# feiyue126/find_circ2

Measured on AMD Instinct MI355X. Metric: anchor-pairs/sec (backsplice calls) at 100 bp reads, 1/2/4/8 MI355X, higher is better.
Workload: dtype u32

## Files before the change

### find_circ2_amd/csrc/fc2_inflate.hip

```cpp
#include <hip/hip_runtime.h>
#include <stdint.h>
#include <string.h>

#include <algorithm>
#include <atomic>
#include <mutex>
#include <string>
#include <vector>

#include "../../include/fc2_ingest.h"
#include "fc2_common.h"
#include "fc2_devcrc.h"
#include "fc2_inflate.h"

namespace {

constexpr uint32_t kOutMax = 65536;
constexpr uint32_t kRing = 16384;
constexpr uint32_t kRingMask = kRing - 1;
constexpr uint32_t kFlush = 4096;
constexpr int kLitBits = 9;
constexpr int kDistBits = 7;

enum : uint32_t { INF_OK = 0, INF_BAD_TYPE = 1, INF_BAD_STORED = 2, INF_BAD_COUNTS = 3, INF_BAD_CODE = 4,
                  INF_BAD_DIST = 5, INF_OVERFLOW = 6, INF_OVERRUN = 7, INF_SHORT = 8, INF_TOO_BIG = 9,
                  INF_BAD_CLCODE = 10, INF_BAD_CLSYM = 11, INF_BAD_REPEAT = 12, INF_NO_EOB = 13,
                  INF_BAD_LITCODE = 14, INF_BAD_DISTCODE = 15, INF_BAD_CRC = 16 };

enum : uint32_t { K_LIT = 0, K_LEN = 1, K_EOB = 2, K_BAD = 3 };
enum Table { T_LIT, T_DIST, T_CL };

__device__ __forceinline__ uint32_t entry(uint32_t len, uint32_t extra, uint32_t kind, uint32_t value) {
    return len | (extra << 4) | (kind << 8) | (value << 16);
}

struct Lds {
    uint8_t ring[kRing];
    uint32_t lfast[1 << kLitBits];
    uint32_t dfast[1 << kDistBits];
    uint32_t cnt[16];
    uint16_t lsym[288], dsym[32];
    uint8_t lens[320];
};

__constant__ uint16_t kLBase[29] = {3, 4, 5, 6, 7, 8, 9, 10, 11, 13, 15, 17, 19, 23, 27, 31, 35, 43, 51, 59,
                                    67, 83, 99, 115, 131, 163, 195, 227, 258};
__constant__ uint8_t kLExt[29] = {0, 0, 0, 0, 0, 0, 0, 0, 1, 1, 1, 1, 2, 2, 2, 2, 3, 3, 3, 3, 4, 4, 4, 4, 5, 5, 5, 5, 0};
__constant__ uint16_t kDBase[30] = {1, 2, 3, 4, 5, 7, 9, 13, 17, 25, 33, 49, 65, 97, 129, 193, 257, 385, 513, 769,
                                    1025, 1537, 2049, 3073, 4097, 6145, 8193, 12289, 16385, 24577};
__constant__ uint8_t kDExt[30] = {0, 0, 0, 0, 1, 1, 2, 2, 3, 3, 4, 4, 5, 5, 6, 6, 7, 7, 8, 8, 9, 9, 10, 10, 11, 11,
                                  12, 12, 13, 13};
__constant__ uint8_t kClOrder[19] = {16, 17, 18, 0, 8, 7, 9, 6, 10, 5, 11, 4, 12, 3, 13, 2, 14, 1, 15};

__device__ __forceinline__ uint32_t meaning(Table t, uint32_t s, uint32_t len) {
    if (t == T_CL) return entry(len, 0, K_LIT, s);
    if (t == T_DIST) return s < 30 ? entry(len, kDExt[s], K_LEN, kDBase[s]) : entry(len, 0, K_BAD, 0);
    if (s < 256) return entry(len, 0, K_LIT, s);
    if (s == 256) return entry(len, 0, K_EOB, 0);
    return s < 286 ? entry(len, kLExt[s - 257], K_LEN, kLBase[s - 257]) : entry(len, 0, K_BAD, 0);
}

__device__ __forceinline__ uint32_t uni(uint32_t v) { return (uint32_t)__builtin_amdgcn_readfirstlane((int)v); }

struct Bits {
    const uint32_t *w;
    uint32_t pos, end;
    uint64_t bb;
    int nb;
    uint32_t wi;
    uint32_t base, last;
    uint32_t win, nxt;
    int lane;
};

__device__ __forceinline__ uint32_t load_word(const Bits &b, uint32_t k) { return k <= b.last ? b.w[k] : 0u; }
__device__ __forceinline__ void window(Bits &b, uint32_t base) {
    b.base = base;
    b.win = load_word(b, base + (uint32_t)b.lane);
    b.nxt = load_word(b, base + 64u + (uint32_t)b.lane);
}
__device__ __forceinline__ uint32_t word(Bits &b, uint32_t k) {
    if (k - b.base >= 64u) {
        if (k - b.base < 128u) {
            b.base += 64u;
            b.win = b.nxt;
            b.nxt = load_word(b, b.base + 64u + (uint32_t)b.lane);
        } else {
            window(b, k & ~63u);
        }
    }
    return (uint32_t)__builtin_amdgcn_readlane((int)b.win, (int)(k - b.base));
}
__device__ __forceinline__ void seek(Bits &b, uint32_t bitpos) {
    b.pos = bitpos;
    b.wi = bitpos >> 5;
    const uint32_t sh = bitpos & 31u;
    const uint32_t lo = word(b, b.wi);
    const uint32_t hi = word(b, b.wi + 1);
    b.bb = ((uint64_t)lo | ((uint64_t)hi << 32)) >> sh;
    b.nb = 64 - (int)sh;
    b.wi += 2;
}
__device__ __forceinline__ uint32_t peek(Bits &b) {
    if (b.nb <= 32) {
        b.bb |= (uint64_t)word(b, b.wi++) << b.nb;
        b.nb += 32;
    }
    return (uint32_t)b.bb;
}
__device__ __forceinline__ void drop(Bits &b, int n) {
    b.bb >>= n;
    b.nb -= n;
    b.pos += (uint32_t)n;
}
__device__ __forceinline__ uint32_t bits(Bits &b, int n) {
    const uint32_t v = peek(b) & ((1u << n) - 1u);
    drop(b, n);
    return v;
}

struct CodeV {
    uint32_t cnt, first, index;
};

template <int F>
__device__ __forceinline__ uint32_t decode(Bits &b, const uint32_t *fast, const CodeV &cv, const uint16_t *sym, Table t,
                                           uint32_t &val) {
    const uint32_t v = peek(b);
    uint32_t e = uni(fast[v & ((1u << F) - 1u)]);
    if (!(e & 15u)) {
        e = 0;
        const uint32_t rv = __builtin_bitreverse32(v);
        for (int l = F + 1; l <= 15; ++l) {
            const uint32_t code = rv >> (32 - l);
            const uint32_t f = (uint32_t)__builtin_amdgcn_readlane((int)cv.first, l);
            if (code - f < (uint32_t)__builtin_amdgcn_readlane((int)cv.cnt, l)) {
                const uint32_t k = (uint32_t)__builtin_amdgcn_readlane((int)cv.index, l) + code - f;
                e = meaning(t, uni(sym[k]), (uint32_t)l);
                break;
            }
        }
        if (!e) return 0;
    }
    const int cl = (int)(e & 15u), ex = (int)((e >> 4) & 15u);
    val = (e >> 16) + ((uint32_t)(b.bb >> cl) & ((1u << ex) - 1u));
    drop(b, cl + ex);
    return e;
}

template <int F>
__device__ bool build(const uint8_t *lens, int n, uint32_t *fast, uint32_t *cnt, uint16_t *sym, Table t, int lane,
                      CodeV &cv) {
    if (lane < 16) cnt[lane] = 0;
    for (int i = lane; i < (1 << F); i += 64) fast[i] = 0;
    __syncthreads();
    for (int s = lane; s < n; s += 64) {
        const uint32_t l = lens[s];
        if (l) atomicAdd(&cnt[l], 1u);
    }
    __syncthreads();
    uint32_t cnt_v = lane < 16 ? cnt[lane] : 0u;
    cnt_v = lane == 0 ? 0u : cnt_v;
    cv.cnt = cnt_v;
    uint32_t start[16], next[16];
    int left = 1;
    uint32_t idx = 0, code = 0;
#pragma unroll
    for (int l = 1; l < 16; ++l) {
        const uint32_t nl = (uint32_t)__builtin_amdgcn_readlane((int)cnt_v, l);
        const uint32_t np = (uint32_t)__builtin_amdgcn_readlane((int)cnt_v, l - 1);
        left = (left << 1) - (int)nl;
        code = (code + np) << 1;
        start[l] = idx;
        next[l] = code;
        if (lane == l) {
            cv.first = code;
            cv.index = idx;
        }
        idx += nl;
    }
    const uint32_t n1 = (uint32_t)__builtin_amdgcn_readlane((int)cnt_v, 1);
    if (left < 0 || (left > 0 && idx > n1)) {
        __syncthreads();
        return false;
    }
    for (int base = 0; base < n; base += 64) {
        const int s = base + lane;
        const uint32_t l = s < n ? lens[s] : 0u;
#pragma unroll
        for (int ll = 1; ll < 16; ++ll) {
            const uint64_t m = __ballot(l == (uint32_t)ll);
            if (!m) continue;
            if (l == (uint32_t)ll) {
                const uint32_t r = (uint32_t)__popcll(m & ((1ull << lane) - 1ull));
                sym[start[ll] + r] = (uint16_t)s;
                if (ll <= F) {
                    const uint32_t c = next[ll] + r;
                    const uint32_t rev = __builtin_bitreverse32(c) >> (32 - ll);
                    const uint32_t e = meaning(t, (uint32_t)s, (uint32_t)ll);
                    for (uint32_t k = rev; k < (1u << F); k += 1u << ll) fast[k] = e;
                }
            }
            const uint32_t c = (uint32_t)__popcll(m);
            start[ll] += c;
            next[ll] += c;
        }
    }
    __syncthreads();
    return true;
}

__device__ void flush(const Lds &L, uint8_t *dst, uint32_t &flushed, uint32_t upto, bool all, int lane, uint32_t &R) {
    __syncthreads();
    const uint32_t limit = all ? upto : flushed + (upto - flushed) / kFlush * kFlush;
    const uint32_t o = 16u * (uint32_t)lane;
    while (limit - flushed >= 1024u) {
        const uint4 v = *reinterpret_cast<const uint4 *>(L.ring + (flushed & kRingMask) + o);
        *reinterpret_cast<uint4 *>(dst + flushed + o) = v;
        const uint32_t c = crc_word(crc_word(crc_word(crc_word(0u, v.x), v.y), v.z), v.w);
        R = multmodp(kX2n[13], R) ^ wave_fold(c);
        flushed += 1024u;
    }
    if (all && upto > flushed) {
        const uint32_t t = upto - flushed, r = flushed & kRingMask;
        if (o < t) *reinterpret_cast<uint4 *>(dst + flushed + o) = *reinterpret_cast<const uint4 *>(L.ring + r + o);
        for (uint32_t i = 0; i < t; ++i) {
            R ^= uni(L.ring[r + i]);
#pragma unroll
            for (int b = 0; b < 8; ++b) R = mulx(R);
        }
        flushed = upto;
    }
    __threadfence_block();
}

__global__ __launch_bounds__(64) void inflate_kernel(const uint8_t *__restrict__ src, const uint32_t *__restrict__ off,
                                                     const uint32_t *__restrict__ len,
                                                     const uint32_t *__restrict__ isize,
                                                     const uint32_t *__restrict__ crc, uint8_t *__restrict__ dst,
                                                     uint32_t *__restrict__ status) {
    extern __shared__ __align__(16) uint8_t smem[];
    Lds &L = *reinterpret_cast<Lds *>(smem);
    const uint32_t blk = blockIdx.x;
    const int lane = (int)threadIdx.x;
    const uint32_t o = off[blk], want = isize[blk];
    uint8_t *out = dst + (uint64_t)blk * kOutMax;
    uint32_t st = INF_OK;
    if (want > kOutMax || len[blk] >= (1u << 28)) st = INF_TOO_BIG;
    const uint32_t n = st == INF_OK ? len[blk] : 0u;
    Bits b;
    b.w = reinterpret_cast<const uint32_t *>(src + (o & ~3u));
    b.end = (o & 3u) * 8u + n * 8u;
    b.last = ((o & 3u) + n) >> 2;
    b.lane = lane;
    window(b, 0);
    seek(b, (o & 3u) * 8u);
    uint32_t p = 0, flushed = 0;
    uint32_t R = 0;
    CodeV lcv = {0, 0, 0}, dcv = {0, 0, 0};
    bool last = false;
    while (st == INF_OK && !last) {
        if (b.pos + 3 > b.end) { st = INF_OVERRUN; break; }
        last = bits(b, 1) != 0;
        const uint32_t type = bits(b, 2);
        if (type == 0) {
            seek(b, (b.pos + 7u) & ~7u);
            if (b.pos + 32 > b.end) { st = INF_OVERRUN; break; }
            const uint32_t sl = bits(b, 16), nl = bits(b, 16);
            if (sl != (~nl & 0xFFFFu)) { st = INF_BAD_STORED; break; }
            if (b.pos + sl * 8u > b.end) { st = INF_OVERRUN; break; }
            if (p + sl > want) { st = INF_OVERFLOW; break; }
            const uint8_t *s = reinterpret_cast<const uint8_t *>(b.w) + (b.pos >> 3);
            for (uint32_t done = 0; done < sl;) {
                const uint32_t k = min(sl - done, kFlush);
                for (uint32_t j = (uint32_t)lane; j < k; j += 64) L.ring[(p + j) & kRingMask] = s[done + j];
                p += k;
                done += k;
                if (p - flushed >= kFlush) flush(L, out, flushed, p, false, lane, R);
            }
            seek(b, b.pos + sl * 8u);
            continue;
        }
        if (type == 3) { st = INF_BAD_TYPE; break; }
        if (type == 1) {
            for (int s = lane; s < 288 + 32; s += 64)
                L.lens[s] = (uint8_t)(s < 144 ? 8 : s < 256 ? 9 : s < 280 ? 7 : s < 288 ? 8 : 5);
            __syncthreads();
            if (!build<kLitBits>(L.lens, 288, L.lfast, L.cnt, L.lsym, T_LIT, lane, lcv) ||
                !build<kDistBits>(L.lens + 288, 32, L.dfast, L.cnt, L.dsym, T_DIST, lane, dcv)) {
                st = INF_BAD_LITCODE;
                break;
            }
        } else {
            if (b.pos + 14 > b.end) { st = INF_OVERRUN; break; }
            const int nlen = (int)bits(b, 5) + 257, ndist = (int)bits(b, 5) + 1, ncode = (int)bits(b, 4) + 4;
            if (nlen > 286 || ndist > 30) { st = INF_BAD_COUNTS; break; }
            if (lane < 19) L.lens[lane] = 0;
            __syncthreads();
            for (int k = 0; k < ncode; ++k) {
                const uint32_t v = bits(b, 3);
                if (lane == 0) L.lens[kClOrder[k]] = (uint8_t)v;
            }
            __syncthreads();
            if (!build<7>(L.lens, 19, L.dfast, L.cnt, L.dsym, T_CL, lane, dcv)) { st = INF_BAD_CLCODE; break; }
            const int total = nlen + ndist;
            int k = 0;
            while (k < total) {
                if (b.pos > b.end) { st = INF_OVERRUN; break; }
                uint32_t sym;
                if (!decode<7>(b, L.dfast, dcv, L.dsym, T_CL, sym)) { st = INF_BAD_CLSYM; break; }
                if (sym < 16) {
                    if (lane == 0) L.lens[k] = (uint8_t)sym;
                    ++k;
                    continue;
                }
                uint32_t val = 0;
                int rep;
                if (sym == 16) {
                    if (k == 0) { st = INF_BAD_REPEAT; break; }
                    __syncthreads();
                    val = uni(L.lens[k - 1]);
                    rep = 3 + (int)bits(b, 2);
                } else if (sym == 17) {
                    rep = 3 + (int)bits(b, 3);
                } else {
                    rep = 11 + (int)bits(b, 7);
                }
                if (k + rep > total) { st = INF_BAD_REPEAT; break; }
                for (int r = lane; r < rep; r += 64) L.lens[k + r] = (uint8_t)val;
                k += rep;
            }
            if (st != INF_OK) break;
            if (b.pos > b.end) { st = INF_OVERRUN; break; }
            __syncthreads();
            if (uni(L.lens[256]) == 0) { st = INF_NO_EOB; break; }
            if (!build<kLitBits>(L.lens, nlen, L.lfast, L.cnt, L.lsym, T_LIT, lane, lcv)) {
                st = INF_BAD_LITCODE;
                break;
            }
            if (!build<kDistBits>(L.lens + nlen, ndist, L.dfast, L.cnt, L.dsym, T_DIST, lane, dcv)) {
                st = INF_BAD_DISTCODE;
                break;
            }
        }
        for (;;) {
            if (b.pos > b.end) { st = INF_OVERRUN; break; }
            uint32_t val;
            const uint32_t e = decode<kLitBits>(b, L.lfast, lcv, L.lsym, T_LIT, val);
            const uint32_t kind = (e >> 8) & 0xFFu;
            if (!e || kind == K_BAD) { st = INF_BAD_CODE; break; }
            if (kind == K_LIT) {
                if (p >= want) { st = INF_OVERFLOW; break; }
                if (lane == 0) L.ring[p & kRingMask] = (uint8_t)val;
                ++p;
            } else if (kind == K_EOB) {
                break;
            } else {
                const uint32_t mlen = val;
                uint32_t dist;
                const uint32_t de = decode<kDistBits>(b, L.dfast, dcv, L.dsym, T_DIST, dist);
                if (!de || ((de >> 8) & 0xFFu) == K_BAD || dist > p) { st = INF_BAD_DIST; break; }
                if (p + mlen > want) { st = INF_OVERFLOW; break; }
                if (dist + mlen <= kRing) {
                    for (uint32_t j = (uint32_t)lane; j < mlen; j += 64)
                        L.ring[(p + j) & kRingMask] = L.ring[(p - dist + (j < dist ? j : j % dist)) & kRingMask];
                } else {
                    for (uint32_t j = (uint32_t)lane; j < mlen; j += 64)
                        L.ring[(p + j) & kRingMask] = out[p - dist + (j < dist ? j : j % dist)];
                }
                p += mlen;
            }
            if (p - flushed >= kFlush) flush(L, out, flushed, p, false, lane, R);
        }
    }
    if (st == INF_OK && p != want) st = INF_SHORT;
    if (st == INF_OK && b.pos > b.end) st = INF_OVERRUN;
    if (st == INF_OK) {
        flush(L, out, flushed, p, true, lane, R);
        if (crc && (R ^ multmodp(x8n(want), 0xFFFFFFFFu) ^ 0xFFFFFFFFu) != crc[blk]) st = INF_BAD_CRC;
    }
    if (lane == 0) status[blk] = st;
}

__global__ __launch_bounds__(256) void compact_kernel(const uint8_t *__restrict__ slots, const uint32_t *__restrict__ isize,
                                                      const uint32_t *__restrict__ ooff,
                                                      const uint32_t *__restrict__ status, uint8_t *__restrict__ out) {
    const uint32_t blk = blockIdx.y;
    const uint32_t b0 = 16u * (blockIdx.x * 256u + threadIdx.x);
    const uint32_t n = isize[blk];
    if (status[blk] != INF_OK || b0 >= n) return;
    const uint4 v = *reinterpret_cast<const uint4 *>(slots + (uint64_t)blk * kOutMax + b0);
    uint8_t *d = out + ooff[blk] + b0;
    if (b0 + 16u <= n && ((uintptr_t)d & 15u) == 0) {
        *reinterpret_cast<uint4 *>(d) = v;
        return;
    }
    const uint32_t w[4] = {v.x, v.y, v.z, v.w};
    const uint32_t k = min(16u, n - b0);
    for (uint32_t i = 0; i < k; ++i) d[i] = (uint8_t)(w[i >> 2] >> (8u * (i & 3u)));
}


constexpr uint32_t kWalkCap = FC2_BAM_WALK_CAP;
static_assert((kOutMax - 4) / 36 + 1 <= kWalkCap, "a block's record starts fit a row");

__device__ __forceinline__ uint32_t walk_u32(const uint32_t *__restrict__ w, uint32_t o) {
    const uint32_t i = o >> 2, s = (o & 3u) * 8u;
    const uint32_t lo = w[i];
    if (!s) return lo;
    return (lo >> s) | (w[i + 1] << (32u - s));
}

__device__ bool walk_plausible(const uint32_t *__restrict__ w, uint32_t o, uint32_t n) {
    if (o > n || n - o < 36u) return false;
    const uint32_t avail = n - o;
    const int32_t bs = (int32_t)walk_u32(w, o);
    if (bs < 32 || bs >= (1 << 28)) return false;
    const int32_t ref = (int32_t)walk_u32(w, o + 4), pos = (int32_t)walk_u32(w, o + 8);
    const uint32_t lname = walk_u32(w, o + 12) & 0xFFu, ncig = walk_u32(w, o + 16) & 0xFFFFu;
    const int32_t lseq = (int32_t)walk_u32(w, o + 20), nref = (int32_t)walk_u32(w, o + 24),
                  npos = (int32_t)walk_u32(w, o + 28);
    if (ref < -1 || pos < -1 || lname < 1 || lseq < 0 || nref < -1 || npos < -1) return false;
    if (32ull + lname + 4ull * ncig + ((uint64_t)lseq + 1) / 2 + (uint64_t)lseq > (uint64_t)bs) return false;
    if (36u + lname > avail) return true;
    const uint8_t *p = reinterpret_cast<const uint8_t *>(w) + o + 36u;
    if (p[lname - 1] != 0) return false;
    for (uint32_t k = 0; k + 1 < lname; ++k)
        if (p[k] < 0x21 || p[k] > 0x7e) return false;
    return true;
}

__global__ __launch_bounds__(64) void bam_walk_kernel(const uint8_t *__restrict__ slots, const uint32_t *__restrict__ isize,
                                                      const uint32_t *__restrict__ status, uint16_t *__restrict__ starts,
                                                      uint32_t *__restrict__ count, uint32_t *__restrict__ exit_at) {
    const uint32_t blk = blockIdx.x, lane = threadIdx.x;
    if (status && status[blk] != INF_OK) {
        if (lane == 0) count[blk] = 0, exit_at[blk] = FC2_BAM_WALK_NO_EXIT;
        return;
    }
    const uint32_t n = min(isize[blk], kOutMax);
    const uint32_t *w = reinterpret_cast<const uint32_t *>(slots + (uint64_t)blk * kOutMax);
    uint16_t *row = starts + (uint64_t)blk * kWalkCap;
    uint32_t o = FC2_BAM_WALK_NO_EXIT;
    for (uint32_t b = 0; b + 36u <= n; b += 64u) {
        const uint32_t c = b + lane;
        bool ok = walk_plausible(w, c, n);
        if (ok) {
            const uint32_t nx = c + 4u + walk_u32(w, c);
            ok = nx + 36u > n || walk_plausible(w, nx, n);
        }
        const unsigned long long m = __ballot(ok);
        if (m) {
            o = b + (uint32_t)__ffsll(m) - 1u;
            break;
        }
    }
    o = uni(o);
    uint32_t cnt = 0, ex = FC2_BAM_WALK_NO_EXIT;
    if (o != FC2_BAM_WALK_NO_EXIT) {
        bool cut = false;
        while (cnt < kWalkCap && o + 4u <= n) {
            const int32_t bs = (int32_t)uni(walk_u32(w, o));
            if (bs < 32) { cut = true; break; }
            if (lane == 0) row[cnt] = (uint16_t)o;
            ++cnt;
            o += 4u + (uint32_t)bs;
        }
        if (!cut) ex = o;
    }
    if (lane == 0) count[blk] = cnt, exit_at[blk] = ex;
}


constexpr uint32_t kDigestMaxBlocks = FC2_BAM_DIGEST_MAX_BLOCKS;
static_assert(sizeof(fc2_bam_digest) == 32, "a digest row is 32 bytes");

__device__ __forceinline__ uint32_t dg_u8(const uint8_t *__restrict__ b, uint64_t o) { return b[o]; }
__device__ __forceinline__ uint32_t dg_u16(const uint8_t *__restrict__ b, uint64_t o) {
    return dg_u8(b, o) | (dg_u8(b, o + 1) << 8);
}
__device__ __forceinline__ uint32_t dg_u32(const uint8_t *__restrict__ b, uint64_t o) {
    return dg_u8(b, o) | (dg_u8(b, o + 1) << 8) | (dg_u8(b, o + 2) << 16) | (dg_u8(b, o + 3) << 24);
}

__device__ __forceinline__ uint32_t dg_tag_bits(const uint8_t *__restrict__ b, uint64_t p, uint32_t ty) {
    switch (ty) {
        case 'c': return (uint32_t)(int32_t)(int8_t)dg_u8(b, p);
        case 'C': return dg_u8(b, p);
        case 's': return (uint32_t)(int32_t)(int16_t)dg_u16(b, p);
        case 'S': return dg_u16(b, p);
        case 'i': case 'I': case 'f': return dg_u32(b, p);
        default: return 0;
    }
}

__device__ bool digest_record(const uint8_t *__restrict__ bytes, uint32_t n_bytes, uint64_t at,
                              const uint32_t *__restrict__ ooff, const uint32_t *__restrict__ status, uint32_t blk,
                              uint32_t n_blocks, fc2_bam_digest &r) {
    if (at + 4 > n_bytes) return false;
    const uint32_t bs = dg_u32(bytes, at);
    r.block_size = bs;
    if (bs < 32u || bs >= (1u << 28)) return false;
    const uint64_t b = at + 4, lim = b + bs;
    if (lim > n_bytes) return false;
    if (status)
        for (uint32_t j = blk; j < n_blocks && (j == blk || ooff[j] < lim); ++j)
            if (status[j] != INF_OK) return false;
    const int64_t pos = (int32_t)dg_u32(bytes, b + 4);
    const uint32_t l_name = dg_u8(bytes, b + 8), n_cig = dg_u16(bytes, b + 12), flag = dg_u16(bytes, b + 14);
    const int64_t l_seq = (int32_t)dg_u32(bytes, b + 16);
    if (l_seq < 0 || 32 + (int64_t)l_name + 4 * (int64_t)n_cig + (l_seq + 1) / 2 + l_seq > (int64_t)bs) return false;
    if (l_name == 0 || dg_u8(bytes, b + 32 + l_name - 1) != 0) return false;
    uint64_t p = b + 32 + l_name;
    uint64_t ref_span = 0, astart = 0, lead = 0, trail = 0;
    bool stop = false, leading = true;
    for (uint32_t k = 0; k < n_cig; ++k, p += 4) {
        const uint32_t c = dg_u32(bytes, p), op = c & 0xFu, len = c >> 4;
        if (op == 0 || op == 2 || op == 3 || op == 7 || op == 8) ref_span += len;
        if (!stop) {
            if (op == 4 || op == 5) astart += len;
            else if (op == 0) stop = true;
        }
        if (leading) {
            if (op == 4) lead += len;
            else if (op != 5) leading = false;
        }
        if (op == 4) trail += len;
        else if (op != 5) trail = 0;
    }
    if ((ref_span | astart | lead | trail) >> 31) return false;
    r.astart = (int32_t)astart;
    r.aend = ((flag & 4u) || n_cig == 0) ? -1 : pos + (int64_t)ref_span;
    if (l_seq > 0) {
        const int64_t n = l_seq;
        int64_t s0 = (int64_t)lead, e0 = n - (int64_t)trail;
        if (e0 < 0) e0 += n;
        s0 = s0 > n ? n : s0;
        e0 = e0 < 0 ? 0 : (e0 > n ? n : e0);
        r.qlen = (int32_t)(e0 > s0 ? e0 - s0 : 0);
        r.has_qual = dg_u8(bytes, p + (uint64_t)(l_seq + 1) / 2) != 0xFFu;
    } else {
        r.qlen = -1;
        r.has_qual = 0;
    }
    p += (uint64_t)(l_seq + 1) / 2 + (uint64_t)l_seq;
    uint32_t n_as = 0, n_xs = 0;
    while (p < lim) {
        if (lim - p < 3) return false;
        const uint32_t t0 = dg_u8(bytes, p), t1 = dg_u8(bytes, p + 1), ty = dg_u8(bytes, p + 2);
        p += 3;
        const uint64_t left = lim - p;
        uint64_t n;
        switch (ty) {
            case 'c': case 'C': case 'A': n = 1; break;
            case 's': case 'S': n = 2; break;
            case 'i': case 'I': case 'f': n = 4; break;
            case 'Z': case 'H': {
                uint64_t z = p;
                while (z < lim && dg_u8(bytes, z) != 0) ++z;
                if (z == lim) return false;
                n = z - p + 1;
                break;
            }
            case 'B': {
                if (left < 5) return false;
                const uint32_t sub = dg_u8(bytes, p);
                const uint32_t w = (sub == 'c' || sub == 'C') ? 1u : (sub == 's' || sub == 'S') ? 2u
                                 : (sub == 'i' || sub == 'I' || sub == 'f') ? 4u : 0u;
                const int32_t cnt = (int32_t)dg_u32(bytes, p + 1);
                if (!w || cnt < 0) return false;
                n = 5 + (uint64_t)w * (uint32_t)cnt;
                break;
            }
            default: return false;
        }
        if (n > left) return false;
        const bool as = t0 == 'A' && t1 == 'S', xs = t0 == 'X' && t1 == 'S';
        if (as) {
            if (n_as++) return false;
            r.as_type = (uint8_t)ty;
            r.as_bits = dg_tag_bits(bytes, p, ty);
        }
        if (xs) {
            if (n_xs++) return false;
            r.xs_type = (uint8_t)ty;
            r.xs_bits = dg_tag_bits(bytes, p, ty);
        }
        p += n;
    }
    return true;
}

__global__ __launch_bounds__(64) void bam_digest_kernel(const uint8_t *__restrict__ bytes, uint32_t n_bytes,
                                                        const uint32_t *__restrict__ ooff, const uint32_t *__restrict__ status,
                                                        const uint16_t *__restrict__ starts, const uint32_t *__restrict__ count,
                                                        fc2_bam_digest *__restrict__ rows, uint32_t *__restrict__ first,
                                                        uint32_t n_blocks) {
    const uint32_t blk = blockIdx.x, lane = threadIdx.x;
    uint32_t f = 0;
    for (uint32_t j = lane; j < blk; j += 64u) f += min(count[j], kWalkCap);
    for (int d = 32; d; d >>= 1) f += __shfl_xor(f, d, 64);
    const uint32_t cnt = min(count[blk], kWalkCap);
    if (lane == 0) {
        first[blk] = f;
        if (blk + 1 == n_blocks) first[n_blocks] = f + cnt;
    }
    const uint16_t *row = starts + (uint64_t)blk * kWalkCap;
    const uint32_t o0 = ooff[blk];
    for (uint32_t k = lane; k < cnt; k += 64u) {
        fc2_bam_digest r;
        r.state = r.as_type = r.xs_type = r.has_qual = 0;
        r.block_size = 0;
        r.astart = r.qlen = 0;
        r.as_bits = r.xs_bits = 0;
        r.aend = 0;
        if (digest_record(bytes, n_bytes, (uint64_t)o0 + row[k], ooff, status, blk, n_blocks, r)) {
            r.state = 1;
        } else {
            const uint32_t bs = r.block_size;
            r.as_type = r.xs_type = r.has_qual = 0;
            r.astart = r.qlen = 0;
            r.as_bits = r.xs_bits = 0;
            r.aend = 0;
            r.block_size = bs;
        }
        rows[(uint64_t)f + k] = r;
    }
}

}

extern "C" int fc2_bam_digest_launch(const uint8_t *bytes, uint32_t n_bytes, const uint32_t *ooff, const uint32_t *isize,
                                     const uint32_t *status, const uint16_t *starts, const uint32_t *count,
                                     fc2_bam_digest *rows, uint32_t *first, uint32_t n_blocks, void *stream) {
    if (!n_blocks) return FC2_OK;
    if ((!bytes && n_bytes) || !ooff || !isize || !starts || !count || !rows || !first)
        return fc2::fail(FC2_E_PARAM, "fc2_bam_digest_launch: null argument");
    if (n_blocks > kDigestMaxBlocks) return fc2::fail(FC2_E_PARAM, "fc2_bam_digest_launch: more than 1024 blocks");
    if (((uintptr_t)rows & 7u) || ((uintptr_t)first & 3u))
        return fc2::fail(FC2_E_PARAM, "fc2_bam_digest_launch: rows must be 8-byte and first 4-byte aligned");
    hipLaunchKernelGGL(bam_digest_kernel, dim3(n_blocks), dim3(64), 0, (hipStream_t)stream, bytes, n_bytes, ooff, status,
                       starts, count, rows, first, n_blocks);
    const hipError_t e = hipGetLastError();
    return e == hipSuccess ? FC2_OK : fc2::fail(FC2_E_HIP, std::string("fc2_bam_digest_launch: ") + hipGetErrorString(e));
}

extern "C" int fc2_bam_walk_launch(const uint8_t *slots, const uint32_t *isize, const uint32_t *status, uint16_t *starts,
                                   uint32_t *count, uint32_t *exit, uint32_t n_blocks, void *stream) {
    if (!n_blocks) return FC2_OK;
    if (!slots || !isize || !starts || !count || !exit) return fc2::fail(FC2_E_PARAM, "fc2_bam_walk_launch: null argument");
    if ((uintptr_t)slots & 3u) return fc2::fail(FC2_E_PARAM, "fc2_bam_walk_launch: slots must be 4-byte aligned");
    hipLaunchKernelGGL(bam_walk_kernel, dim3(n_blocks), dim3(64), 0, (hipStream_t)stream, slots, isize, status, starts,
                       count, exit);
    const hipError_t e = hipGetLastError();
    return e == hipSuccess ? FC2_OK : fc2::fail(FC2_E_HIP, std::string("fc2_bam_walk_launch: ") + hipGetErrorString(e));
}

extern "C" int fc2_bgzf_inflate_launch(const uint8_t *src, const uint32_t *off, const uint32_t *len,
                                       const uint32_t *isize, const uint32_t *crc, uint8_t *dst, uint32_t *status,
                                       uint32_t n, void *stream) {
    if (!n) return FC2_OK;
    if (!src || !off || !len || !isize || !dst || !status) return fc2::fail(FC2_E_PARAM, "fc2_bgzf_inflate_launch: null argument");
    static bool attr = [] {
        return hipFuncSetAttribute(reinterpret_cast<const void *>(inflate_kernel),
                                   hipFuncAttributeMaxDynamicSharedMemorySize, (int)sizeof(Lds)) == hipSuccess;
    }();
    if (!attr) return fc2::fail(FC2_E_HIP, "fc2_bgzf_inflate_launch: cannot reserve the kernel's LDS");
    hipLaunchKernelGGL(inflate_kernel, dim3(n), dim3(64), sizeof(Lds), (hipStream_t)stream, src, off, len, isize, crc,
                       dst, status);
    const hipError_t e = hipGetLastError();
    return e == hipSuccess ? FC2_OK : fc2::fail(FC2_E_HIP, std::string("fc2_bgzf_inflate_launch: ") + hipGetErrorString(e));
}

namespace fc2 {
namespace inf {

namespace {
struct Pool {
    struct Buf {
        void *p;
        size_t size;
    };
    std::mutex mu;
    size_t cap = 0;
    int users = 0, max_buffers = 0;
    std::vector<Buf> idle, all;
};
Pool &pool() {
    static Pool *p = new Pool();
    return *p;
}
std::atomic<bool> pool_on{false};

void pool_open(size_t cap, int max_buffers) {
    Pool &P = pool();
    std::lock_guard<std::mutex> g(P.mu);
    ++P.users;
    P.cap = std::max(P.cap, cap);
    P.max_buffers = std::max(P.max_buffers, max_buffers);
    pool_on = true;
}
void pool_drop(Pool &P, void *b) {
    (void)hipHostFree(b);
    for (size_t k = 0; k < P.all.size(); ++k)
        if (P.all[k].p == b) {
            P.all.erase(P.all.begin() + (ptrdiff_t)k);
            break;
        }
}
void pool_close() {
    Pool &P = pool();
    std::lock_guard<std::mutex> g(P.mu);
    if (--P.users > 0) return;
    pool_on = false;
    for (const Pool::Buf &b : P.idle) pool_drop(P, b.p);
    P.idle.clear();
    P.cap = 0;
    P.max_buffers = 0;
}
}

void *pinned_take(size_t n) {
    if (!pool_on.load(std::memory_order_relaxed)) return nullptr;
    Pool &P = pool();
    std::lock_guard<std::mutex> g(P.mu);
    if (!P.users || n > P.cap) return nullptr;
    for (size_t k = 0; k < P.idle.size(); ++k)
        if (P.idle[k].size >= n) {
            void *b = P.idle[k].p;
            P.idle.erase(P.idle.begin() + (ptrdiff_t)k);
            return b;
        }
    if ((int)P.all.size() >= P.max_buffers) return nullptr;
    void *b = nullptr;
    if (hipHostMalloc(&b, P.cap, hipHostMallocDefault) != hipSuccess) return nullptr;
    P.all.push_back({b, P.cap});
    return b;
}

bool pinned_owns(const void *b) {
    Pool &P = pool();
    std::lock_guard<std::mutex> g(P.mu);
    for (const Pool::Buf &x : P.all)
        if (x.p == b) return true;
    return false;
}

bool pinned_give(void *b) {
    Pool &P = pool();
    std::lock_guard<std::mutex> g(P.mu);
    for (const Pool::Buf &x : P.all)
        if (x.p == b) {
            if (P.users) P.idle.push_back(x);
            else pool_drop(P, b);
            return true;
        }
    return false;
}

constexpr int kStreams = 4;

struct Gpu {
    int device = 0;
    uint32_t max_blocks = 0;
    size_t src_cap = 0;
    hipStream_t stream[kStreams] = {};
    hipEvent_t done[kStreams] = {};
    uint8_t *h_src = nullptr, *d_src = nullptr, *d_slots = nullptr, *d_out = nullptr;
    uint32_t *h_meta = nullptr, *d_meta = nullptr;
    uint32_t *h_walk = nullptr, *d_walk = nullptr;
    uint16_t *h_starts = nullptr, *d_starts = nullptr;
    bool walk = false;
    fc2_bam_digest *d_rows = nullptr, *h_rows = nullptr;
    uint32_t *d_first = nullptr, *h_first = nullptr;
    size_t rows_cap = 0;
    struct Chunk {
        uint32_t i0, c, foff;
        int s;
        uint64_t row0;
    };
    std::vector<Chunk> dchunks;
    bool digest = false, digest_ok = false, rows_ready = false;
    bool pooled = false;
    char *dest = nullptr;
    uint32_t n = 0;
    uint64_t out = 0;
    int chunks = 0;
    bool ok = true;
    std::string err;
};

static bool hip_ok(Gpu *g, hipError_t e, const char *what) {
    if (e == hipSuccess) return true;
    if (g->ok) g->err = std::string("GPU inflate: ") + what + ": " + hipGetErrorString(e);
    g->ok = false;
    return false;
}

Gpu *gpu_open(int device, uint32_t max_blocks, size_t pool_cap, std::string &err) {
    Gpu *g = new Gpu();
    g->device = device;
    g->max_blocks = max_blocks;
    g->src_cap = (size_t)max_blocks * kOutMax + 64;
    const size_t out = (size_t)max_blocks * kOutMax, meta = (size_t)max_blocks * 7 * sizeof(uint32_t);
    const size_t walk = (size_t)max_blocks * 2 * sizeof(uint32_t), rows = (size_t)max_blocks * kWalkCap * sizeof(uint16_t);
    bool ok = hip_ok(g, hipSetDevice(device), "hipSetDevice");
    for (int k = 0; k < kStreams && ok; ++k)
        ok = hip_ok(g, hipStreamCreateWithFlags(&g->stream[k], hipStreamNonBlocking), "stream") &&
             hip_ok(g, hipEventCreateWithFlags(&g->done[k], hipEventBlockingSync | hipEventDisableTiming), "event");
    ok = ok && hip_ok(g, hipHostMalloc((void **)&g->h_src, g->src_cap, hipHostMallocDefault), "pinned input") &&
         hip_ok(g, hipHostMalloc((void **)&g->h_meta, meta, hipHostMallocDefault), "pinned table") &&
         hip_ok(g, hipMalloc((void **)&g->d_src, g->src_cap), "device input") &&
         hip_ok(g, hipMalloc((void **)&g->d_slots, out), "device slots") &&
         hip_ok(g, hipMalloc((void **)&g->d_out, out), "device output") &&
         hip_ok(g, hipMalloc((void **)&g->d_meta, meta), "device table") &&
         hip_ok(g, hipHostMalloc((void **)&g->h_walk, walk, hipHostMallocDefault), "pinned record counts") &&
         hip_ok(g, hipHostMalloc((void **)&g->h_starts, rows, hipHostMallocDefault), "pinned record lists") &&
         hip_ok(g, hipMalloc((void **)&g->d_walk, walk), "device record counts") &&
         hip_ok(g, hipMalloc((void **)&g->d_starts, rows), "device record lists");
    if (!ok) {
        err = g->err;
        gpu_close(g);
        return nullptr;
    }
    if (pool_cap) {
        pool_open(pool_cap, 16);
        g->pooled = true;
        void *first[3];
        for (void *&b : first) b = pinned_take(pool_cap);
        for (void *b : first)
            if (b) pinned_give(b);
    }
    return g;
}

void gpu_close(Gpu *g) {
    if (!g) return;
    if (hipSetDevice(g->device) == hipSuccess) {
        for (int k = 0; k < kStreams; ++k)
            if (g->stream[k]) (void)hipStreamSynchronize(g->stream[k]);
        if (g->d_first) (void)hipFree(g->d_first);
        if (g->d_rows) (void)hipFree(g->d_rows);
        if (g->h_first) (void)hipHostFree(g->h_first);
        if (g->h_rows) (void)hipHostFree(g->h_rows);
        if (g->d_starts) (void)hipFree(g->d_starts);
        if (g->d_walk) (void)hipFree(g->d_walk);
        if (g->h_starts) (void)hipHostFree(g->h_starts);
        if (g->h_walk) (void)hipHostFree(g->h_walk);
        if (g->d_meta) (void)hipFree(g->d_meta);
        if (g->d_out) (void)hipFree(g->d_out);
        if (g->d_slots) (void)hipFree(g->d_slots);
        if (g->d_src) (void)hipFree(g->d_src);
        if (g->h_meta) (void)hipHostFree(g->h_meta);
        if (g->h_src) (void)hipHostFree(g->h_src);
        for (int k = 0; k < kStreams; ++k) {
            if (g->done[k]) (void)hipEventDestroy(g->done[k]);
            if (g->stream[k]) (void)hipStreamDestroy(g->stream[k]);
        }
    }
    if (g->pooled) pool_close();
    delete g;
}

uint32_t gpu_max_blocks(const Gpu *g) { return g->max_blocks; }

constexpr size_t kRowsPerBlock = 512;

void gpu_begin(Gpu *g, char *dest, bool walk, bool digest) {
    g->dest = dest;
    g->walk = walk;
    g->digest = walk && digest;
    g->digest_ok = g->digest;
    g->rows_ready = false;
    g->dchunks.clear();
    g->n = 0;
    g->out = 0;
    g->chunks = 0;
    g->ok = hipSetDevice(g->device) == hipSuccess;
    g->err = g->ok ? "" : "GPU inflate: hipSetDevice failed";
    if (g->ok && g->digest && !g->d_rows) {
        const size_t M = g->max_blocks;
        g->rows_cap = M * kRowsPerBlock;
        hip_ok(g, hipMalloc((void **)&g->d_rows, M * kWalkCap * sizeof(fc2_bam_digest)), "device digest rows") &&
            hip_ok(g, hipMalloc((void **)&g->d_first, (2 * M + 1) * sizeof(uint32_t)), "device row index") &&
            hip_ok(g, hipHostMalloc((void **)&g->h_rows, g->rows_cap * sizeof(fc2_bam_digest), hipHostMallocDefault),
                   "pinned digest rows") &&
            hip_ok(g, hipHostMalloc((void **)&g->h_first, (2 * M + 1) * sizeof(uint32_t), hipHostMallocDefault),
                   "pinned row index");
    }
}

bool gpu_add(Gpu *g, const uint8_t *raw, const size_t *boff, const size_t *bsz, size_t i0, size_t i1) {
    if (!g->ok) return false;
    if (i1 <= i0) return true;
    if (i0 != g->n || i1 > g->max_blocks || boff[i1 - 1] + bsz[i1 - 1] + 8 > g->src_cap) {
        g->ok = false;
        g->err = "GPU inflate: chunk out of order or larger than the buffers";
        return false;
    }
    const uint32_t M = g->max_blocks;
    uint32_t *off = g->h_meta, *len = off + M, *isz = len + M, *crc = isz + M, *ooff = crc + M, *st = ooff + M,
             *rooff = st + M;
    const size_t b0 = boff[i0], b1 = boff[i1 - 1] + bsz[i1 - 1];
    memcpy(g->h_src + b0, raw + b0, b1 - b0);
    memset(g->h_src + b1, 0, 8);
    bool fits = true;
    for (size_t i = i0; i < i1; ++i) {
        const uint8_t *b = raw + boff[i];
        const size_t xl = b[10] | (b[11] << 8);
        off[i] = (uint32_t)(boff[i] + 12 + xl);
        len[i] = (uint32_t)(bsz[i] - 12 - xl - 8);
        const uint8_t *t = b + bsz[i] - 8;
        crc[i] = t[0] | (t[1] << 8) | (t[2] << 16) | ((uint32_t)t[3] << 24);
        isz[i] = t[4] | (t[5] << 8) | (t[6] << 16) | ((uint32_t)t[7] << 24);
        ooff[i] = (uint32_t)g->out;
        rooff[i] = ooff[i] - ooff[i0];
        if (isz[i] > kOutMax) fits = false;
        g->out += std::min<uint32_t>(isz[i], kOutMax);
    }
    g->n = (uint32_t)i1;
    const uint32_t c = (uint32_t)(i1 - i0);
    if (!fits) {
        for (size_t i = i0; i < i1; ++i) st[i] = INF_TOO_BIG;
        g->digest_ok = false;
        return true;
    }
    hipStream_t s = g->stream[g->chunks++ % kStreams];
    uint32_t *d_off = g->d_meta, *d_len = d_off + M, *d_isz = d_len + M, *d_crc = d_isz + M, *d_ooff = d_crc + M,
             *d_st = d_ooff + M;
    const size_t w = sizeof(uint32_t);
    bool ok = hip_ok(g, hipMemcpyAsync(g->d_src + b0, g->h_src + b0, b1 + 8 - b0, hipMemcpyHostToDevice, s), "upload");
    for (int a = 0; a < 5 && ok; ++a)
        ok = hip_ok(g, hipMemcpyAsync(g->d_meta + (size_t)a * M + i0, g->h_meta + (size_t)a * M + i0, c * w,
                                      hipMemcpyHostToDevice, s), "upload");
    ok = ok && fc2_bgzf_inflate_launch(g->d_src, d_off + i0, d_len + i0, d_isz + i0, d_crc + i0,
                                       g->d_slots + (size_t)i0 * kOutMax, d_st + i0, c, s) == FC2_OK;
    if (!ok) {
        if (g->ok) g->err = "GPU inflate: launch failed";
        g->ok = false;
        return false;
    }
    hipLaunchKernelGGL(compact_kernel, dim3(kOutMax / 16 / 256, c), dim3(256), 0, s, g->d_slots + (size_t)i0 * kOutMax,
                       d_isz + i0, d_ooff + i0, d_st + i0, g->d_out);
    const uint64_t o0 = ooff[i0];
    if (!hip_ok(g, hipGetLastError(), "compact")) return false;
    if (g->walk) {
        if (fc2_bam_walk_launch(g->d_slots + (size_t)i0 * kOutMax, d_isz + i0, d_st + i0, g->d_starts + (size_t)i0 * kWalkCap,
                                g->d_walk + i0, g->d_walk + M + i0, c, s) != FC2_OK) {
            if (g->ok) g->err = "GPU inflate: record list launch failed";
            g->ok = false;
            return false;
        }
        ok = hip_ok(g, hipMemcpyAsync(g->h_starts + (size_t)i0 * kWalkCap, g->d_starts + (size_t)i0 * kWalkCap,
                                      (size_t)c * kWalkCap * sizeof(uint16_t), hipMemcpyDeviceToHost, s), "download") &&
             hip_ok(g, hipMemcpyAsync(g->h_walk + i0, g->d_walk + i0, c * w, hipMemcpyDeviceToHost, s), "download") &&
             hip_ok(g, hipMemcpyAsync(g->h_walk + M + i0, g->d_walk + M + i0, c * w, hipMemcpyDeviceToHost, s), "download");
        if (!ok) return false;
    }
    if (g->digest && g->digest_ok && c <= kDigestMaxBlocks) {
        Gpu::Chunk ch{(uint32_t)i0, c, (uint32_t)(i0 + g->dchunks.size()), (int)((g->chunks - 1) % kStreams), 0};
        uint32_t *d_rooff = d_st + M;
        ok = hip_ok(g, hipMemcpyAsync(d_rooff + i0, rooff + i0, c * w, hipMemcpyHostToDevice, s), "upload");
        if (ok && fc2_bam_digest_launch(g->d_out + o0, (uint32_t)(g->out - o0), d_rooff + i0, d_isz + i0, d_st + i0,
                                        g->d_starts + (size_t)i0 * kWalkCap, g->d_walk + i0,
                                        g->d_rows + (size_t)i0 * kWalkCap, g->d_first + ch.foff, c, s) != FC2_OK) {
            if (g->ok) g->err = "GPU inflate: record digest launch failed";
            g->ok = false;
            return false;
        }
        ok = ok && hip_ok(g, hipMemcpyAsync(g->h_first + ch.foff, g->d_first + ch.foff, (c + 1) * w, hipMemcpyDeviceToHost, s),
                          "download");
        if (!ok) return false;
        g->dchunks.push_back(ch);
    }
    return hip_ok(g, hipMemcpyAsync(g->dest + o0, g->d_out + o0, g->out - o0, hipMemcpyDeviceToHost, s), "download") &&
           hip_ok(g, hipMemcpyAsync(st + i0, d_st + i0, c * w, hipMemcpyDeviceToHost, s), "download");
}

bool gpu_finish(Gpu *g, std::string &err) {
    for (int k = 0; k < kStreams; ++k)
        if (hip_ok(g, hipEventRecord(g->done[k], g->stream[k]), "event")) hip_ok(g, hipEventSynchronize(g->done[k]), "kernel");
    if (g->ok && g->digest && g->digest_ok && !g->dchunks.empty()) {
        uint64_t total = 0;
        for (Gpu::Chunk &ch : g->dchunks) {
            ch.row0 = total;
            total += std::min<uint64_t>(g->h_first[ch.foff + ch.c], (uint64_t)ch.c * kWalkCap);
        }
        if (total <= g->rows_cap) {
            bool used[kStreams] = {};
            for (const Gpu::Chunk &ch : g->dchunks) {
                const uint64_t n = std::min<uint64_t>(g->h_first[ch.foff + ch.c], (uint64_t)ch.c * kWalkCap);
                if (n && hip_ok(g, hipMemcpyAsync(g->h_rows + ch.row0, g->d_rows + (size_t)ch.i0 * kWalkCap,
                                                  n * sizeof(fc2_bam_digest), hipMemcpyDeviceToHost, g->stream[ch.s]), "download"))
                    used[ch.s] = true;
            }
            for (int k = 0; k < kStreams; ++k)
                if (used[k] && hip_ok(g, hipEventRecord(g->done[k], g->stream[k]), "event"))
                    hip_ok(g, hipEventSynchronize(g->done[k]), "download");
            g->rows_ready = g->ok;
        }
    }
    if (!g->ok) err = g->err;
    return g->ok;
}

uint32_t gpu_status(const Gpu *g, size_t i) { return g->h_meta[5 * (size_t)g->max_blocks + i]; }

const uint16_t *gpu_walk(const Gpu *g, size_t i, uint32_t &count, uint32_t &exit) {
    count = std::min<uint32_t>(g->h_walk[i], kWalkCap);
    exit = g->h_walk[(size_t)g->max_blocks + i];
    return g->h_starts + i * kWalkCap;
}

const fc2_bam_digest *gpu_digest(const Gpu *g, size_t i, uint32_t &count) {
    count = 0;
    if (!g->rows_ready) return nullptr;
    for (const Gpu::Chunk &ch : g->dchunks)
        if (i >= ch.i0 && i < ch.i0 + ch.c) {
            const uint32_t *f = g->h_first + ch.foff;
            const uint32_t a = f[i - ch.i0], b = f[i - ch.i0 + 1];
            if (a > b || b > f[ch.c] || (uint64_t)f[ch.c] > (uint64_t)ch.c * kWalkCap) return nullptr;
            count = b - a;
            return g->h_rows + ch.row0 + a;
        }
    return nullptr;
}

}
}
```

Baseline: 24.42 billion.

## Speculatively decode symbols at every bit offset across the wave in inflate

Each of the 64 lanes now decodes a literal/length plus distance symbol at a different bit offset of a shared window. A serial readlane walk then chains the valid records, so a run of literals and short non-overlapping matches is committed in one batched LDS write instead of one symbol per iteration. Anything unusual (long codes that are not literals, overlapping or long matches, EOB, or data near the end of the stream) falls back to the original scalar decode path through a seek. The change also turns the build() per-length arrays into lane registers and adds a fast copy path for short non-overlapping matches. These reduce serial per-symbol overhead in the single-wave inflate kernel, at the cost of more register pressure and wasted speculative lookups.

Measured after the change: 24.41 billion (median of 2 runs). About the same (-0.0%).

```diff
diff --git a/find_circ2_amd/csrc/fc2_inflate.hip b/find_circ2_amd/csrc/fc2_inflate.hip
--- a/find_circ2_amd/csrc/fc2_inflate.hip
+++ b/find_circ2_amd/csrc/fc2_inflate.hip
@@ -21,6 +21,14 @@
 constexpr uint32_t kFlush = 4096;
 constexpr int kLitBits = 9;
 constexpr int kDistBits = 7;
+
+#ifndef FC2_INFLATE_WINDOW
+#define FC2_INFLATE_WINDOW 1
+#endif
+#if FC2_INFLATE_WINDOW
+constexpr uint32_t kLitFlag = 1u << 16;
+enum : uint32_t { W_PAIR = 1u << 6, W_CLEAN = 1u << 7 };
+#endif
 
 enum : uint32_t { INF_OK = 0, INF_BAD_TYPE = 1, INF_BAD_STORED = 2, INF_BAD_COUNTS = 3, INF_BAD_CODE = 4,
                   INF_BAD_DIST = 5, INF_OVERFLOW = 6, INF_OVERRUN = 7, INF_SHORT = 8, INF_TOO_BIG = 9,
@@ -79,7 +87,8 @@
     b.win = load_word(b, base + (uint32_t)b.lane);
     b.nxt = load_word(b, base + 64u + (uint32_t)b.lane);
 }
-__device__ __forceinline__ uint32_t word(Bits &b, uint32_t k) {
+__device__ __forceinline__ void advance(Bits &b) {
+    const uint32_t k = b.pos >> 5;
     if (k - b.base >= 64u) {
         if (k - b.base < 128u) {
             b.base += 64u;
@@ -89,10 +98,27 @@
             window(b, k & ~63u);
         }
     }
+}
+__device__ __forceinline__ uint32_t word(Bits &b, uint32_t k) {
+    const uint32_t i = k - b.base;
+    if (i < 64u) return (uint32_t)__builtin_amdgcn_readlane((int)b.win, (int)i);
+    if (i < 128u) return (uint32_t)__builtin_amdgcn_readlane((int)b.nxt, (int)(i - 64u));
+    window(b, k & ~63u);
     return (uint32_t)__builtin_amdgcn_readlane((int)b.win, (int)(k - b.base));
 }
+#if FC2_INFLATE_WINDOW
+__device__ __forceinline__ uint32_t near_word(const Bits &b, uint32_t i) {
+    const uint32_t a = (uint32_t)__builtin_amdgcn_readlane((int)b.win, (int)(i & 63u));
+    const uint32_t c = (uint32_t)__builtin_amdgcn_readlane((int)b.nxt, (int)(i & 63u));
+    return i < 64u ? a : c;
+}
+__device__ __forceinline__ uint32_t funnel(uint32_t lo, uint32_t hi, uint32_t r) {
+    return (uint32_t)((((uint64_t)hi << 32) | lo) >> r);
+}
+#endif
 __device__ __forceinline__ void seek(Bits &b, uint32_t bitpos) {
     b.pos = bitpos;
+    advance(b);
     b.wi = bitpos >> 5;
     const uint32_t sh = bitpos & 31u;
     const uint32_t lo = word(b, b.wi);
@@ -118,10 +144,23 @@
     drop(b, n);
     return v;
 }
-
 struct CodeV {
     uint32_t cnt, first, index;
 };
+
+template <int F>
+__device__ __forceinline__ uint32_t long_code(uint32_t v, const CodeV &cv, const uint16_t *sym) {
+    const uint32_t rv = __builtin_bitreverse32(v);
+    for (int l = F + 1; l <= 15; ++l) {
+        const uint32_t code = rv >> (32 - l);
+        const uint32_t f = (uint32_t)__builtin_amdgcn_readlane((int)cv.first, l);
+        if (code - f < (uint32_t)__builtin_amdgcn_readlane((int)cv.cnt, l)) {
+            const uint32_t k = (uint32_t)__builtin_amdgcn_readlane((int)cv.index, l) + code - f;
+            return ((uint32_t)l << 16) | uni(sym[k]);
+        }
+    }
+    return 0;
+}
 
 template <int F>
 __device__ __forceinline__ uint32_t decode(Bits &b, const uint32_t *fast, const CodeV &cv, const uint16_t *sym, Table t,
@@ -129,18 +168,9 @@
     const uint32_t v = peek(b);
     uint32_t e = uni(fast[v & ((1u << F) - 1u)]);
     if (!(e & 15u)) {
-        e = 0;
-        const uint32_t rv = __builtin_bitreverse32(v);
-        for (int l = F + 1; l <= 15; ++l) {
-            const uint32_t code = rv >> (32 - l);
-            const uint32_t f = (uint32_t)__builtin_amdgcn_readlane((int)cv.first, l);
-            if (code - f < (uint32_t)__builtin_amdgcn_readlane((int)cv.cnt, l)) {
-                const uint32_t k = (uint32_t)__builtin_amdgcn_readlane((int)cv.index, l) + code - f;
-                e = meaning(t, uni(sym[k]), (uint32_t)l);
-                break;
-            }
-        }
-        if (!e) return 0;
+        const uint32_t lc = long_code<F>(v, cv, sym);
+        if (!lc) return 0;
+        e = meaning(t, lc & 0xFFFFu, lc >> 16);
     }
     const int cl = (int)(e & 15u), ex = (int)((e >> 4) & 15u);
     val = (e >> 16) + ((uint32_t)(b.bb >> cl) & ((1u << ex) - 1u));
@@ -149,8 +179,8 @@
 }
 
 template <int F>
-__device__ bool build(const uint8_t *lens, int n, uint32_t *fast, uint32_t *cnt, uint16_t *sym, Table t, int lane,
-                      CodeV &cv) {
+__device__ __forceinline__ bool build(const uint8_t *lens, int n, uint32_t *fast, uint32_t *cnt, uint16_t *sym, Table t,
+                                      int lane, CodeV &cv) {
     if (lane < 16) cnt[lane] = 0;
     for (int i = lane; i < (1 << F); i += 64) fast[i] = 0;
     __syncthreads();
@@ -162,7 +192,7 @@
     uint32_t cnt_v = lane < 16 ? cnt[lane] : 0u;
     cnt_v = lane == 0 ? 0u : cnt_v;
     cv.cnt = cnt_v;
-    uint32_t start[16], next[16];
+    uint32_t start = 0, next = 0;
     int left = 1;
     uint32_t idx = 0, code = 0;
 #pragma unroll
@@ -171,11 +201,9 @@
         const uint32_t np = (uint32_t)__builtin_amdgcn_readlane((int)cnt_v, l - 1);
         left = (left << 1) - (int)nl;
         code = (code + np) << 1;
-        start[l] = idx;
-        next[l] = code;
         if (lane == l) {
-            cv.first = code;
-            cv.index = idx;
+            cv.first = next = code;
+            cv.index = start = idx;
         }
         idx += nl;
     }
@@ -191,19 +219,23 @@
         for (int ll = 1; ll < 16; ++ll) {
             const uint64_t m = __ballot(l == (uint32_t)ll);
             if (!m) continue;
+            const uint32_t s0 = (uint32_t)__builtin_amdgcn_readlane((int)start, ll);
+            const uint32_t c0 = (uint32_t)__builtin_amdgcn_readlane((int)next, ll);
             if (l == (uint32_t)ll) {
                 const uint32_t r = (uint32_t)__popcll(m & ((1ull << lane) - 1ull));
-                sym[start[ll] + r] = (uint16_t)s;
+                sym[s0 + r] = (uint16_t)s;
                 if (ll <= F) {
-                    const uint32_t c = next[ll] + r;
+                    const uint32_t c = c0 + r;
                     const uint32_t rev = __builtin_bitreverse32(c) >> (32 - ll);
                     const uint32_t e = meaning(t, (uint32_t)s, (uint32_t)ll);
                     for (uint32_t k = rev; k < (1u << F); k += 1u << ll) fast[k] = e;
                 }
             }
-            const uint32_t c = (uint32_t)__popcll(m);
-            start[ll] += c;
-            next[ll] += c;
+            if (lane == ll) {
+                const uint32_t c = (uint32_t)__popcll(m);
+                start += c;
+                next += c;
+            }
         }
     }
     __syncthreads();
@@ -232,6 +264,24 @@
         flushed = upto;
     }
     __threadfence_block();
+}
+
+__device__ __forceinline__ void copy_match(Lds &L, const uint8_t *out, uint32_t p, uint32_t mlen, uint32_t dist, int lane) {
+    const uint32_t j0 = (uint32_t)lane;
+    if (dist >= mlen && dist + mlen <= kRing) {
+        if (mlen <= 64u) {
+            const uint8_t c = L.ring[(p - dist + j0) & kRingMask];
+            if (j0 < mlen) L.ring[(p + j0) & kRingMask] = c;
+        } else {
+            for (uint32_t j = j0; j < mlen; j += 64) L.ring[(p + j) & kRingMask] = L.ring[(p - dist + j) & kRingMask];
+        }
+    } else if (dist + mlen <= kRing) {
+        for (uint32_t j = j0; j < mlen; j += 64)
+            L.ring[(p + j) & kRingMask] = L.ring[(p - dist + (j < dist ? j : j % dist)) & kRingMask];
+    } else {
+        for (uint32_t j = j0; j < mlen; j += 64)
+            L.ring[(p + j) & kRingMask] = out[p - dist + (j < dist ? j : j % dist)];
+    }
 }
 
 __global__ __launch_bounds__(64) void inflate_kernel(const uint8_t *__restrict__ src, const uint32_t *__restrict__ off,
@@ -260,6 +310,7 @@
     CodeV lcv = {0, 0, 0}, dcv = {0, 0, 0};
     bool last = false;
     while (st == INF_OK && !last) {
+        advance(b);
         if (b.pos + 3 > b.end) { st = INF_OVERRUN; break; }
         last = bits(b, 1) != 0;
         const uint32_t type = bits(b, 2);
@@ -282,18 +333,15 @@
             continue;
         }
         if (type == 3) { st = INF_BAD_TYPE; break; }
+        int nlen = 288, ndist = 32;
         if (type == 1) {
             for (int s = lane; s < 288 + 32; s += 64)
                 L.lens[s] = (uint8_t)(s < 144 ? 8 : s < 256 ? 9 : s < 280 ? 7 : s < 288 ? 8 : 5);
             __syncthreads();
-            if (!build<kLitBits>(L.lens, 288, L.lfast, L.cnt, L.lsym, T_LIT, lane, lcv) ||
-                !build<kDistBits>(L.lens + 288, 32, L.dfast, L.cnt, L.dsym, T_DIST, lane, dcv)) {
-                st = INF_BAD_LITCODE;
-                break;
-            }
         } else {
             if (b.pos + 14 > b.end) { st = INF_OVERRUN; break; }
-            const int nlen = (int)bits(b, 5) + 257, ndist = (int)bits(b, 5) + 1, ncode = (int)bits(b, 4) + 4;
+            nlen = (int)bits(b, 5) + 257, ndist = (int)bits(b, 5) + 1;
+            const int ncode = (int)bits(b, 4) + 4;
             if (nlen > 286 || ndist > 30) { st = INF_BAD_COUNTS; break; }
             if (lane < 19) L.lens[lane] = 0;
             __syncthreads();
@@ -306,6 +354,7 @@
             const int total = nlen + ndist;
             int k = 0;
             while (k < total) {
+                advance(b);
                 if (b.pos > b.end) { st = INF_OVERRUN; break; }
                 uint32_t sym;
                 if (!decode<7>(b, L.dfast, dcv, L.dsym, T_CL, sym)) { st = INF_BAD_CLSYM; break; }
@@ -334,40 +383,108 @@
             if (b.pos > b.end) { st = INF_OVERRUN; break; }
             __syncthreads();
             if (uni(L.lens[256]) == 0) { st = INF_NO_EOB; break; }
-            if (!build<kLitBits>(L.lens, nlen, L.lfast, L.cnt, L.lsym, T_LIT, lane, lcv)) {
-                st = INF_BAD_LITCODE;
-                break;
+        }
+        if (!build<kLitBits>(L.lens, nlen, L.lfast, L.cnt, L.lsym, T_LIT, lane, lcv)) { st = INF_BAD_LITCODE; break; }
+        if (!build<kDistBits>(L.lens + nlen, ndist, L.dfast, L.cnt, L.dsym, T_DIST, lane, dcv)) {
+            st = INF_BAD_DISTCODE;
+            break;
+        }
+        for (;;) {
+#if FC2_INFLATE_WINDOW
+            advance(b);
+            const uint32_t wi = (b.pos >> 5) - b.base;
+            const uint32_t w0 = near_word(b, wi), w1 = near_word(b, wi + 1), w2 = near_word(b, wi + 2), w3 = near_word(b, wi + 3);
+            const uint32_t o1 = (b.pos & 31u) + (uint32_t)lane, q1 = o1 >> 5;
+            const uint32_t v1 = funnel(q1 == 0 ? w0 : q1 == 1 ? w1 : w2, q1 == 0 ? w1 : q1 == 1 ? w2 : w3, o1 & 31u);
+            const uint32_t le = L.lfast[v1 & ((1u << kLitBits) - 1u)];
+            const uint32_t cl = le & 15u, ex = (le >> 4) & 15u, kind = (le >> 8) & 0xFFu;
+            const uint32_t lv = (le >> 16) + ((v1 >> cl) & ((1u << ex) - 1u));
+            const uint32_t o2 = o1 + cl + ex, q2 = o2 >> 5;
+            const uint32_t v2 = funnel(q2 == 0 ? w0 : q2 == 1 ? w1 : q2 == 2 ? w2 : w3,
+                                       q2 == 0 ? w1 : q2 == 1 ? w2 : q2 == 2 ? w3 : 0u, o2 & 31u);
+            const uint32_t de = L.dfast[v2 & ((1u << kDistBits) - 1u)];
+            const uint32_t dcl = de & 15u, dex = (de >> 4) & 15u;
+            const uint32_t dv = (de >> 16) + ((v2 >> dcl) & ((1u << dex) - 1u));
+            const uint32_t nbits = kind == K_LEN ? cl + ex + dcl + dex : cl;
+            const bool inside = cl != 0 && b.pos + (uint32_t)lane + nbits <= b.end;
+            const bool pair = inside && kind == K_LEN && dcl != 0 && ((de >> 8) & 0xFFu) == K_LEN;
+            const bool clean = (inside && kind == K_LIT) || (pair && lv <= 64u && dv + lv <= kRing && dv <= p);
+            const uint32_t rec0 = (pair || clean ? nbits | ((kind == K_LIT ? 1u : lv) << 8) : 0u) |
+                                  (pair ? W_PAIR : 0u) | (clean ? W_CLEAN : 0u);
+            const uint32_t rec1 = kind == K_LIT ? kLitFlag | lv : dv;
+            const uint32_t room = min(want - p, 64u);
+            uint32_t s = 0, o = 0, src = 0;
+            uint32_t r0 = 0, r1 = 0;
+            bool stopped = false;
+            do {
+                r0 = (uint32_t)__builtin_amdgcn_readlane((int)rec0, (int)s);
+                r1 = (uint32_t)__builtin_amdgcn_readlane((int)rec1, (int)s);
+                if (!(r0 & W_CLEAN)) {
+                    if (!(r0 & W_PAIR) && !((uint32_t)__builtin_amdgcn_readlane((int)cl, (int)s))) {
+                        const uint32_t lc = long_code<kLitBits>((uint32_t)__builtin_amdgcn_readlane((int)v1, (int)s), lcv, L.lsym);
+                        if ((lc & 0xFFFFu) < 256u && lc && b.pos + s + (lc >> 16) <= b.end) {
+                            r0 = (lc >> 16) | (1u << 8) | W_CLEAN;
+                            r1 = kLitFlag | (lc & 0xFFu);
+                        }
+                    }
+                    if (!(r0 & W_CLEAN)) {
+                        stopped = true;
+                        break;
+                    }
+                }
+                const uint32_t t = o + (r0 >> 8);
+                if (t > room || r1 < t) {
+                    stopped = true;
+                    break;
+                }
+                src = (uint32_t)lane >= o ? r1 : src;
+                o = t;
+                s += r0 & 63u;
+            } while (s < 64u);
+            if (o) {
+                const uint32_t at = p + (uint32_t)lane;
+                const uint32_t from = L.ring[(at - src) & kRingMask];
+                if ((uint32_t)lane < o) L.ring[at & kRingMask] = (uint8_t)((src & kLitFlag) ? src : from);
+                p += o;
+                b.pos += s;
             }
-            if (!build<kDistBits>(L.lens + nlen, ndist, L.dfast, L.cnt, L.dsym, T_DIST, lane, dcv)) {
-                st = INF_BAD_DISTCODE;
-                break;
+            bool one = false;
+            if (stopped) {
+                if (r0 & W_PAIR) {
+                    const uint32_t mlen = (r0 >> 8) & 0x1FFu;
+                    if (r1 <= p && p + mlen <= want) {
+                        copy_match(L, out, p, mlen, r1, lane);
+                        p += mlen;
+                        b.pos += r0 & 63u;
+                    } else {
+                        one = true;
+                    }
+                } else {
+                    one = !(r0 & W_CLEAN) || p >= want;
+                }
             }
-        }
-        for (;;) {
+            if (p - flushed >= kFlush) flush(L, out, flushed, p, false, lane, R);
+            if (!one) continue;
+            seek(b, b.pos);
+#endif
             if (b.pos > b.end) { st = INF_OVERRUN; break; }
             uint32_t val;
             const uint32_t e = decode<kLitBits>(b, L.lfast, lcv, L.lsym, T_LIT, val);
-            const uint32_t kind = (e >> 8) & 0xFFu;
-            if (!e || kind == K_BAD) { st = INF_BAD_CODE; break; }
-            if (kind == K_LIT) {
+            const uint32_t ekind = (e >> 8) & 0xFFu;
+            if (!e || ekind == K_BAD) { st = INF_BAD_CODE; break; }
+            if (ekind == K_LIT) {
                 if (p >= want) { st = INF_OVERFLOW; break; }
                 if (lane == 0) L.ring[p & kRingMask] = (uint8_t)val;
                 ++p;
-            } else if (kind == K_EOB) {
+            } else if (ekind == K_EOB) {
                 break;
             } else {
                 const uint32_t mlen = val;
                 uint32_t dist;
-                const uint32_t de = decode<kDistBits>(b, L.dfast, dcv, L.dsym, T_DIST, dist);
-                if (!de || ((de >> 8) & 0xFFu) == K_BAD || dist > p) { st = INF_BAD_DIST; break; }
+                const uint32_t dd = decode<kDistBits>(b, L.dfast, dcv, L.dsym, T_DIST, dist);
+                if (!dd || ((dd >> 8) & 0xFFu) == K_BAD || dist > p) { st = INF_BAD_DIST; break; }
                 if (p + mlen > want) { st = INF_OVERFLOW; break; }
-                if (dist + mlen <= kRing) {
-                    for (uint32_t j = (uint32_t)lane; j < mlen; j += 64)
-                        L.ring[(p + j) & kRingMask] = L.ring[(p - dist + (j < dist ? j : j % dist)) & kRingMask];
-                } else {
-                    for (uint32_t j = (uint32_t)lane; j < mlen; j += 64)
-                        L.ring[(p + j) & kRingMask] = out[p - dist + (j < dist ? j : j % dist)];
-                }
+                copy_match(L, out, p, mlen, dist, lane);
                 p += mlen;
             }
             if (p - flushed >= kFlush) flush(L, out, flushed, p, false, lane, R);
```
